# levendlee/np-modeling

Measured on AMD Instinct MI355X. Metric: fwd+bwd samples/sec, TransformerEncoder d=1024 seq=512, higher is better.
Workload: dtype f32; 1 GPU; TransformerEncoder fwd+bwd+SGD step, d_model=1024, heads=8, seq=512, hidden_units=4096, pre-norm, batch 256/GPU (BASELINE.json configs[4] per-GPU shard; global batch 256); global_batch=256, seq_len=512, parallelism=single GPU

## Files before the change

np_modeling_amd/csrc/npm_attn.hip:

```cpp
#include <algorithm>
#include <cmath>
#include <cstring>

#include "npm_mfma_tile.h"

namespace {

using npm_tile::f32x16;
using npm_tile::xcd_remap;

constexpr float LOG2E = 1.44269504088896340736f;
constexpr float LN2 = 0.69314718055994530942f;
constexpr int OOB = 0x7FFFFFFF;

struct MhaArgs {
    const float *q, *k, *v;
    long q_pitch, k_pitch, v_pitch;
    float *ctx;
    long ctx_pitch;
    float *lse;
    float *delta;
    long delta_sb, delta_sh;
    int delta_len;
    float *lse2;
    int sq_pad;
    const unsigned char *skip;
    long skip_sb, skip_sh;
    int skip_nkb;
    long skip_all;
    const float *dctx;
    long dctx_pitch;
    float *dq, *dk, *dv;
    long dq_pitch, dk_pitch, dv_pitch;
    const unsigned char *mask;
    long mask_sb, mask_sh, mask_sq;
    float *scores;
    int batch, heads, seq_q, seq_kv;
    int kv_heads;
    float scale;
    int q_tiles;
    int q_pair;
    int stagger;
    long long *trace;
};

template <int D>
struct Tile {
    static constexpr int CPR = D / 4;
    static constexpr int SWZ = (CPR < 16 ? CPR : 16) - 1;
    __host__ __device__ static constexpr int sw(int row) {
        return D >= 64 ? ((row & 15) ^ ((row & 4) << 1))
             : D == 32 ? (((row >> 1) & 1) | (((row >> 3) & 1) << 1) | (((row >> 2) & 1) << 2))
                       : (((row >> 3) & 1) << 1);
    }
    __host__ __device__ static constexpr int prow(int row) { return D <= 32 ? row ^ ((row >> 2) & 1) : row; }
    static constexpr int PIECE_ROWS = 256 / D;
    static constexpr int NG = D / 8;
    static constexpr int NB = NG < 8 ? NG : 8;
    static_assert(D == 16 || D == 32 || D == 64 || D == 128 || D == 256, "head dim (256: the dS tile of a 256-key block)");
    __device__ static __forceinline__ int chunk(int row, int c) { return prow(row) * D + ((c ^ sw(row)) << 2); }
    __device__ static __forceinline__ int elem(int row, int col) { return prow(row) * D + ((((col >> 2) ^ sw(row)) << 2) | (col & 3)); }
    __device__ static __forceinline__ unsigned src(int lane, int piece, long pitch) {
        const int row = prow(piece * PIECE_ROWS + lane / CPR);
        const int c = (lane % CPR) ^ sw(row);
        return (unsigned)((row * pitch + c * 4) * 4);
    }
    __device__ static __forceinline__ void row_bases(int l32, int half, int (&rb)[NB]) {
#pragma unroll
        for (int j = 0; j < NB; ++j) rb[j] = chunk(l32, 2 * j + half);
    }
    __device__ static constexpr int row_imm(int g) { return (g >> 3) * 64; }
    static constexpr int VEC = D >= 32 ? D / 32 : 1;
    __device__ static __forceinline__ void vec_bases(int half, int l32, int (&vb)[2][4]) {
        const int col = VEC * (D < 32 ? (l32 & (D - 1)) : l32);
#pragma unroll
        for (int par = 0; par < 2; ++par)
#pragma unroll
            for (int k = 0; k < 4; ++k) vb[par][k] = elem(4 * half + k + 8 * par, col);
    }
    __device__ static constexpr int vec_imm(int r) { return 16 * (r >> 3) * D; }
};

__device__ __forceinline__ float4 ld4(const float *p) { return *reinterpret_cast<const float4 *>(p); }
template <int VEC>
__device__ __forceinline__ void ldv(const float *p, float (&v)[4]) {
    if (VEC == 4) { const float4 x = ld4(p); v[0] = x.x; v[1] = x.y; v[2] = x.z; v[3] = x.w; }
    else if (VEC == 2) { const float2 x = *reinterpret_cast<const float2 *>(p); v[0] = x.x; v[1] = x.y; }
    else v[0] = p[0];
}
__device__ __forceinline__ float ld_stream(const float *p) { return __builtin_nontemporal_load(p); }
__device__ __forceinline__ float xhalf(float x) { return __shfl_xor(x, 32, 64); }
__device__ __forceinline__ float fast_exp2(float x) { return __builtin_amdgcn_exp2f(x); }

typedef unsigned u32x4_t __attribute__((ext_vector_type(4)));

__device__ __forceinline__ float4 buf_load4(__amdgpu_buffer_rsrc_t r, int voff) {
    const u32x4_t v = __builtin_amdgcn_raw_buffer_load_b128(r, voff, 0, 0);
    return make_float4(__uint_as_float(v.x), __uint_as_float(v.y), __uint_as_float(v.z), __uint_as_float(v.w));
}
__device__ __forceinline__ void buf_store4(__amdgpu_buffer_rsrc_t r, int voff, float a, float b, float c, float d) {
    u32x4_t v = {__float_as_uint(a), __float_as_uint(b), __float_as_uint(c), __float_as_uint(d)};
    __builtin_amdgcn_raw_buffer_store_b128(v, r, voff, 0, 0);
}
__device__ __forceinline__ __amdgpu_buffer_rsrc_t make_rsrc(const void *base, long bytes) {
    return __builtin_amdgcn_make_buffer_rsrc((void *)base, 0, (int)std::min<long>(std::max<long>(bytes, 0), 0x7FFFFFF0L), 0x00020000);
}

using npm_tile::i32x4_t;
using npm_tile::make_desc;
using npm_tile::lds_offset;
using npm_tile::dma_group;

#define MFMA(a, b, c) __builtin_amdgcn_mfma_f32_32x32x2f32((a), (b), (c), 0, 0, 0)

template <int STEPS, int READS, int MFMAS>
__device__ __forceinline__ void sched_pipeline() {
    __builtin_amdgcn_sched_group_barrier(0x100, READS, 0);
#pragma unroll
    for (int i = 0; i + 1 < STEPS; ++i) {
        __builtin_amdgcn_sched_group_barrier(0x100, READS, 0);
        __builtin_amdgcn_sched_group_barrier(0x008, MFMAS, 0);
    }
    __builtin_amdgcn_sched_group_barrier(0x008, MFMAS, 0);
}
#define PHASE_END() __builtin_amdgcn_sched_barrier(0)
#define FENCE() __builtin_amdgcn_sched_barrier(0)
#define STAMP(slot) do { if (tr) { FENCE(); tr[slot] = __builtin_amdgcn_s_memtime(); FENCE(); } } while (0)

__device__ __forceinline__ void zero16(f32x16 &x) {
#pragma unroll
    for (int e = 0; e < 16; ++e) x[e] = 0.f;
}

template <int D, bool MASK, bool SAVE, bool TRACE>
__global__ void __launch_bounds__(256, 2)
mha_fwd_kernel(const MhaArgs p) {
    using T = Tile<D>;
    constexpr int NG = D / 8, DT = (D + 31) / 32, VEC = T::VEC, TILE = 32 * D, PIECES = D / 8, PPW = (PIECES + 3) / 4;
    __shared__ __attribute__((aligned(16))) float smem[4 * TILE];

    const int tid = threadIdx.x, lane = tid & 63;
    const int wave = __builtin_amdgcn_readfirstlane(tid >> 6);
    long long *const blk_tr = (TRACE && p.trace && tid == 0) ? p.trace + (long)blockIdx.x * 16 : nullptr;
    if (blk_tr) blk_tr[9] = __builtin_amdgcn_s_memtime();
    const int l32 = lane & 31, half = lane >> 5;

    const int logical = xcd_remap(blockIdx.x, gridDim.x);
    const bool pairing = MASK && p.q_pair;
    const int units = pairing ? (p.q_tiles + 1) / 2 : p.q_tiles;
    const int unit = logical % units, bh = logical / units;
    const int b = bh / p.heads, h = bh - b * p.heads;
  for (int rep = 0; rep < (pairing ? 2 : 1); ++rep) {
    const int qt = rep == 0 ? unit : p.q_tiles - 1 - unit;
    if (rep == 1) {
        if (qt == unit) break;
// ... 672 lines not shown
                    S = MFMA(fa[g & 1].x, fk[g & 1].x, S);
                    S = MFMA(fa[g & 1].y, fk[g & 1].y, S);
                    S = MFMA(fa[g & 1].z, fk[g & 1].z, S);
                    S = MFMA(fa[g & 1].w, fk[g & 1].w, S);
                    FENCE();
                }
            }
            STAMP(1);
            constexpr int F0 = SAVED ? 0 : (NG & 1);
            zero16(dP);
#pragma unroll
            for (int g = 0; g < NG; ++g) {
                if (g + 1 < NG) fa[(F0 + g + 1) & 1] = ld4(tDO + rb[(g + 1) & 7] + T::row_imm(g + 1));
                else ldv<VEC>(tDO + vb[0][0], ea[0]);
                FENCE();
                dP = MFMA(fa[(F0 + g) & 1].x, vf[g].x, dP);
                dP = MFMA(fa[(F0 + g) & 1].y, vf[g].y, dP);
                dP = MFMA(fa[(F0 + g) & 1].z, vf[g].z, dP);
                dP = MFMA(fa[(F0 + g) & 1].w, vf[g].w, dP);
                FENCE();
            }
            unsigned char mk[16];
            if (MASK) {
                const int mvoff = kvok ? kvrow + 4 * half * (int)p.mask_sq : OOB;
#pragma unroll
                for (int r = 0; r < 16; ++r)
                    mk[r] = __builtin_amdgcn_raw_buffer_load_b8(rsrcM, mvoff, (q0 + (r & 3) + 8 * (r >> 2)) * (int)p.mask_sq, 0);
            }
            if (kb * 128 + 128 > p.seq_kv && !kvok) {
#pragma unroll
                for (int r = 0; r < 16; ++r) S[r] = -INFINITY;
            }
#pragma unroll
            for (int r = 0; r < 16; ++r) {
                const float pr = fast_exp2(fmaf((MASK && mk[r] == 0) ? -INFINITY : S[r], c, -Lr[r]));
                P[r] = pr;
                dS[r] = pr * (dP[r] - Dr[r]);
                sDS[ebs[(r >> 2) & 1][r & 3] + 8 * (r >> 2) * 128] = dS[r];
            }
            STAMP(2);
#pragma unroll
            for (int r = 0; r < 16; ++r) {
                if (r + 1 < 16) ldv<VEC>(tDO + vb[((r + 1) >> 2) & 1][(r + 1) & 3] + T::vec_imm(r + 1), ea[(r + 1) & 1]);
                FENCE();
#pragma unroll
                for (int t = 0; t < DT; ++t) dV[t] = MFMA(ea[r & 1][t], P[r], dV[t]);
                FENCE();
            }
            STAMP(3);
            asm volatile("s_waitcnt lgkmcnt(0)" ::: "memory");
            __builtin_amdgcn_s_barrier();
            asm volatile("" ::: "memory");
            STAMP(4);

            if (dq_wave) {
                float4 da[2];
                float dk4[2][4];
                da[0] = ld4(sDS + rbs[0]);
#pragma unroll
                for (int k = 0; k < 4; ++k) dk4[0][k] = sKB[ebk[0][k]];
#pragma unroll
                for (int g = 0; g < 16; ++g) {
                    if (g + 1 < 16) {
                        da[(g + 1) & 1] = ld4(sDS + rbs[(g + 1) & 7] + TS::row_imm(g + 1));
#pragma unroll
                        for (int k = 0; k < 4; ++k) dk4[(g + 1) & 1][k] = sKB[8 * (g + 1) * D + ebk[(g + 1) & 1][k]];
                    } else {
                        ldv<VEC>(tQ + vb[0][0], ea[0]);
                    }
                    if (g == 1) issue_half(nq, nxt, 0);
                    if (g == 9) issue_half(nq, nxt, 1);
                    FENCE();
                    acc = MFMA(dk4[g & 1][0], da[g & 1].x, acc);
                    acc = MFMA(dk4[g & 1][1], da[g & 1].y, acc);
                    acc = MFMA(dk4[g & 1][2], da[g & 1].z, acc);
                    acc = MFMA(dk4[g & 1][3], da[g & 1].w, acc);
                    FENCE();
                }
            } else {
                issue_half(nq, nxt, 0);
                issue_half(nq, nxt, 1);
                ldv<VEC>(tQ + vb[0][0], ea[0]);
            }
            STAMP(5);
            if (seam) {
                __builtin_amdgcn_s_barrier();
                asm volatile("" ::: "memory");
                issue_kblock(kb + 1);
                load_vfrag(kb + 1);
            }
#pragma unroll
            for (int r = 0; r < 16; ++r) {
                if (r + 1 < 16) ldv<VEC>(tQ + vb[((r + 1) >> 2) & 1][(r + 1) & 3] + T::vec_imm(r + 1), ea[(r + 1) & 1]);
                if ((r & 3) == 0 && 8 * (r >> 2) < D) {
                    const int g4 = r >> 2;
                    const u32x4_t v = {__float_as_uint(acc[r]), __float_as_uint(acc[r + 1]), __float_as_uint(acc[r + 2]), __float_as_uint(acc[r + 3])};
                    __builtin_amdgcn_raw_buffer_store_b128(v, rsrcDQw, dq_voff + 32 * g4, dq_tile, 0);
                }
                FENCE();
#pragma unroll
                for (int t = 0; t < DT; ++t) dK[t] = MFMA(ea[r & 1][t], dS[r], dK[t]);
                FENCE();
            }
            if (half == 0) { xs[l32] = lse_n * LOG2E; xs[32 + l32] = dlt_n; }
            in_flight = 4;
            ++it;
            STAMP(6);
            STAMP(7);
            FENCE();
        }
        if (blk_tr && kb == 0) blk_tr[11] = __builtin_amdgcn_s_memtime();
        if (SEAM_STORES == 0) asm volatile("s_waitcnt vmcnt(0)" ::: "memory");
#pragma unroll
        for (int r = 0; r < 16; ++r) {
            const int d0 = VEC * (4 * half + (r & 3) + 8 * (r >> 2));
            if (VEC * (8 * (r >> 2) + (r & 3)) < D) {
                const bool ok = kvok && d0 < D;
                const int offk = ok ? (int)((kvrow * p.dk_pitch + d0) * 4) : OOB, offv = ok ? (int)((kvrow * p.dv_pitch + d0) * 4) : OOB;
                if (VEC == 4) {
                    buf_store4(rsrcDK, offk, dK[0][r], dK[DT > 1 ? 1 : 0][r], dK[DT > 2 ? 2 : 0][r], dK[DT > 3 ? 3 : 0][r]);
                    buf_store4(rsrcDV, offv, dV[0][r], dV[DT > 1 ? 1 : 0][r], dV[DT > 2 ? 2 : 0][r], dV[DT > 3 ? 3 : 0][r]);
                } else {
#pragma unroll
                    for (int t = 0; t < DT; ++t) {
                        __builtin_amdgcn_raw_buffer_store_b32(__float_as_uint(dK[t][r]), rsrcDK, ok ? offk + 4 * t : OOB, 0, 0);
                        __builtin_amdgcn_raw_buffer_store_b32(__float_as_uint(dV[t][r]), rsrcDV, ok ? offv + 4 * t : OOB, 0, 0);
                    }
                }
            }
        }
    }
    if (blk_tr) {
        blk_tr[12] = __builtin_amdgcn_s_memtime();
        asm volatile("s_waitcnt vmcnt(0)" ::: "memory");
        blk_tr[13] = __builtin_amdgcn_s_memtime();
    }
}


template <bool TRACE>
__global__ void __launch_bounds__(512, 1)
mha_bwd16_kernel(const MhaArgs p) {
    constexpr int D = 128;
    using T = Tile<D>;
    constexpr int QTILE = 32 * D, KBLK = 128 * D, ROWS16 = 16 * D;
    __shared__ __attribute__((aligned(16))) float smem[KBLK + 4 * QTILE + 32 * 128];
    float *const sKB = smem, *const sQ = sKB + KBLK, *const sDO = sQ + 2 * QTILE, *const sDS = sDO + 2 * QTILE;

    const int tid = threadIdx.x, lane = tid & 63;
    const int wave = __builtin_amdgcn_readfirstlane(tid >> 6);
    const int l16 = lane & 15, kk = lane >> 4;
    const int bh = blockIdx.x;
    const int b = bh / p.heads, h = bh - b * p.heads;
    long long *const blk_tr = (TRACE && p.trace && tid == 0) ? p.trace + (long)blockIdx.x * 16 : nullptr;
    if (blk_tr) blk_tr[9] = __builtin_amdgcn_s_memtime();

    const auto descK = make_desc(p.k + (long)b * p.seq_kv * p.k_pitch + (h % p.kv_heads) * D, ((long)(p.seq_kv - 1) * p.k_pitch + D) * 4);
    const auto rsrcV = make_rsrc(p.v + (long)b * p.seq_kv * p.v_pitch + (h % p.kv_heads) * D, ((long)(p.seq_kv - 1) * p.v_pitch + D) * 4);
    const auto descQ = make_desc(p.q + (long)b * p.seq_q * p.q_pitch + h * D, ((long)(p.seq_q - 1) * p.q_pitch + D) * 4);
    const auto descDO = make_desc(p.dctx + (long)b * p.seq_q * p.dctx_pitch + h * D, ((long)(p.seq_q - 1) * p.dctx_pitch + D) * 4);
    const auto rsrcDQ = make_rsrc(p.dq + (long)b * p.seq_q * p.dq_pitch + h * D, ((long)(p.seq_q - 1) * p.dq_pitch + D) * 4);
    const auto rsrcDK = make_rsrc(p.dk + (long)b * p.seq_kv * p.dk_pitch + h * D, ((long)(p.seq_kv - 1) * p.dk_pitch + D) * 4);
    const auto rsrcDV = make_rsrc(p.dv + (long)b * p.seq_kv * p.dv_pitch + h * D, ((long)(p.seq_kv - 1) * p.dv_pitch + D) * 4);
    const auto rsrcNone = make_rsrc(p.dq, 0);
    const auto rsrcL = make_rsrc(p.lse2 + (long)bh * p.sq_pad, (long)p.sq_pad * 4);
    const auto rsrcDl = make_rsrc(p.delta + b * p.delta_sb + h * p.delta_sh, (long)p.delta_len * 4);
    const auto rsrcS = make_rsrc(p.scores + (long)bh * p.seq_q * p.seq_kv, (long)p.seq_q * p.seq_kv * 4);
    const int srow_bytes = p.seq_kv * 4;

    unsigned vq[2], vdo[2], vkb[8];
#pragma unroll
    for (int i = 0; i < 2; ++i) {
        vq[i] = T::src(lane, wave * 2 + i, p.q_pitch);
        vdo[i] = T::src(lane, wave * 2 + i, p.dctx_pitch);
    }
#pragma unroll
    for (int i = 0; i < 8; ++i) vkb[i] = T::src(lane, wave * 8 + i, p.k_pitch);
    const unsigned qstep = (unsigned)(32 * p.q_pitch * 4), dostep = (unsigned)(32 * p.dctx_pitch * 4);
    const unsigned lds_q = lds_offset(sQ + wave * 2 * 256), lds_do = lds_offset(sDO + wave * 2 * 256), lds_kb = lds_offset(sKB + wave * 8 * 256);

    int rb[4], vb[4], ws[4];
#pragma unroll
    for (int j = 0; j < 4; ++j) {
        rb[j] = T::chunk(l16, 4 * j + kk);
        vb[j] = T::elem(4 * kk + j, 4 * l16);
        ws[j] = T::elem(4 * kk + j, 16 * wave + l16);
    }

    const float c = p.scale * LOG2E;
    const int nqt = (p.seq_q + 31) / 32, nkb = (p.seq_kv + 127) / 128;
    const int kvl = 16 * wave + l16;
    const int dq_voff = (int)((l16 * p.dq_pitch + 16 * wave + 4 * kk) * 4);
    const int dq_sub = 16 * (int)p.dq_pitch * 4;

    float4 vf[8];
    int it = 0;
    dma_group<8>(descK, lds_kb, 0u, vkb);
    {
        const int row = kvl;
#pragma unroll
        for (int cc = 0; cc < 8; ++cc) {
            vf[cc] = buf_load4(rsrcV, row < p.seq_kv ? (int)((row * p.v_pitch + 16 * cc + 4 * kk) * 4) : OOB);
            vf[cc].x *= p.scale; vf[cc].y *= p.scale; vf[cc].z *= p.scale; vf[cc].w *= p.scale;
        }
    }
    dma_group<2>(descQ, lds_q, 0u, vq);
    dma_group<2>(descDO, lds_do, 0u, vdo);

    bool scale_pending = false;
    f32x4 Lr_n[2], Dr_n[2];
    auto load_rows = [&](int qfirst) {
#pragma unroll
        for (int t = 0; t < 2; ++t) {
            const u32x4_t l4 = __builtin_amdgcn_raw_buffer_load_b128(rsrcL, 16 * kk, (qfirst + 16 * t) * 4, 0);
            const u32x4_t d4 = __builtin_amdgcn_raw_buffer_load_b128(rsrcDl, 16 * kk, (qfirst + 16 * t) * 4, 0);
            Lr_n[t] = f32x4{__uint_as_float(l4.x), __uint_as_float(l4.y), __uint_as_float(l4.z), __uint_as_float(l4.w)};
            Dr_n[t] = f32x4{__uint_as_float(d4.x), __uint_as_float(d4.y), __uint_as_float(d4.z), __uint_as_float(d4.w)};
        }
    };
    load_rows(0);
    if (blk_tr) blk_tr[10] = __builtin_amdgcn_s_memtime();
    for (int kb = 0; kb < nkb; ++kb) {
        const int kvrow = kb * 128 + kvl;
        const bool kvok = kvrow < p.seq_kv;
        f32x4 dK[8], dV[8];
#pragma unroll
        for (int t = 0; t < 8; ++t) { dK[t] = f32x4{0.f, 0.f, 0.f, 0.f}; dV[t] = f32x4{0.f, 0.f, 0.f, 0.f}; }
        const auto rsrcOld = kb > 0 ? rsrcDQ : rsrcNone;
        const int svoff = kvok ? (kvrow + 4 * kk * p.seq_kv) * 4 : OOB;
        int in_flight = kb > 0 ? 18 : 0;

        for (int qt = 0; qt < nqt; ++qt) {
            long long *const tr = (TRACE && blk_tr && kb == (nkb > 1 ? 1 : 0) && qt == (nqt > 5 ? 5 : 0)) ? blk_tr : nullptr;
            STAMP(0);
            if (in_flight == 2) asm volatile("s_waitcnt vmcnt(2) ; npm:wait" ::: "memory");
            else if (in_flight == 18) asm volatile("s_waitcnt vmcnt(18) ; npm:wait" ::: "memory");
            else asm volatile("s_waitcnt vmcnt(0)" ::: "memory");
            asm volatile("s_waitcnt lgkmcnt(0)" ::: "memory");
            __builtin_amdgcn_s_barrier();
            asm volatile("" ::: "memory");
            if (scale_pending) {
#pragma unroll
                for (int cc = 0; cc < 8; ++cc) { vf[cc].x *= p.scale; vf[cc].y *= p.scale; vf[cc].z *= p.scale; vf[cc].w *= p.scale; }
                scale_pending = false;
            }
            STAMP(1);
            const bool seam = qt + 1 == nqt && kb + 1 < nkb;
            const int nq = qt + 1 < nqt ? qt + 1 : 0;
            const int cur = it & 1, nxt = cur ^ 1;
            const float *tQ = sQ + cur * QTILE, *tDO = sDO + cur * QTILE;
            const int q0 = 32 * qt;
            f32x4 Lr[2], Dr[2];
#pragma unroll
            for (int t = 0; t < 2; ++t) { Lr[t] = Lr_n[t]; Dr[t] = Dr_n[t]; }
            load_rows(32 * nq);
            f32x4 S[2], acc[2];
#pragma unroll
            for (int t = 0; t < 2; ++t)
#pragma unroll
                for (int r = 0; r < 4; ++r)
                    S[t][r] = __uint_as_float(__builtin_amdgcn_raw_buffer_load_b32(rsrcS, svoff, (q0 + 16 * t + r) * srow_bytes, 2));
            const int dq_tile = q0 * (int)p.dq_pitch * 4;
#pragma unroll
            for (int t = 0; t < 2; ++t) {
                const u32x4_t o = __builtin_amdgcn_raw_buffer_load_b128(rsrcOld, dq_voff, dq_tile + t * dq_sub, 0);
                acc[t] = f32x4{__uint_as_float(o.x), __uint_as_float(o.y), __uint_as_float(o.z), __uint_as_float(o.w)};
            }

            f32x4 dP[2] = {Dr[0], Dr[1]};
            float4 fa[2][2];
            fa[0][0] = ld4(tDO + rb[0]);
            fa[0][1] = ld4(tDO + rb[0] + ROWS16);
#pragma unroll
            for (int cc = 0; cc < 8; ++cc) {
                if (cc + 1 < 8) {
                    fa[(cc + 1) & 1][0] = ld4(tDO + rb[(cc + 1) & 3] + ((cc + 1) >> 2) * 64);
                    fa[(cc + 1) & 1][1] = ld4(tDO + rb[(cc + 1) & 3] + ((cc + 1) >> 2) * 64 + ROWS16);
                }
                FENCE();
#pragma unroll
                for (int t = 0; t < 2; ++t) {
                    dP[t] = MFMA16(fa[cc & 1][t].x, vf[cc].x, dP[t]);
                    dP[t] = MFMA16(fa[cc & 1][t].y, vf[cc].y, dP[t]);
                    dP[t] = MFMA16(fa[cc & 1][t].z, vf[cc].z, dP[t]);
                    dP[t] = MFMA16(fa[cc & 1][t].w, vf[cc].w, dP[t]);
                }
                FENCE();
            }
            STAMP(2);
            if (kb * 128 + 128 > p.seq_kv && !kvok) {
#pragma unroll
                for (int t = 0; t < 2; ++t)
#pragma unroll
                    for (int r = 0; r < 4; ++r) S[t][r] = -INFINITY;
            }
            f32x4 P[2], dS[2];
#pragma unroll
            for (int t = 0; t < 2; ++t)
#pragma unroll
                for (int r = 0; r < 4; ++r) {
                    const float pr = fast_exp2(fmaf(S[t][r], c, -Lr[t][r]));
                    P[t][r] = pr;
                    dS[t][r] = pr * dP[t][r];
                    sDS[ws[r] + t * ROWS16] = dS[t][r];
                }
            STAMP(3);
            float4 ea[2][2];
            ea[0][0] = ld4(tDO + vb[0]);
            ea[0][1] = ld4(tDO + vb[0] + 64);
#pragma unroll
            for (int st = 0; st < 8; ++st) {
                const int t = st >> 2, r = st & 3;
                if (st + 1 < 8) {
                    ea[(st + 1) & 1][0] = ld4(tDO + vb[(st + 1) & 3] + ((st + 1) >> 2) * ROWS16);
                    ea[(st + 1) & 1][1] = ld4(tDO + vb[(st + 1) & 3] + ((st + 1) >> 2) * ROWS16 + 64);
                }
                FENCE();
                const float4 e0 = ea[st & 1][0], e1 = ea[st & 1][1];
                dV[0] = MFMA16(e0.x, P[t][r], dV[0]); dV[1] = MFMA16(e0.y, P[t][r], dV[1]);
                dV[2] = MFMA16(e0.z, P[t][r], dV[2]); dV[3] = MFMA16(e0.w, P[t][r], dV[3]);
                dV[4] = MFMA16(e1.x, P[t][r], dV[4]); dV[5] = MFMA16(e1.y, P[t][r], dV[5]);
                dV[6] = MFMA16(e1.z, P[t][r], dV[6]); dV[7] = MFMA16(e1.w, P[t][r], dV[7]);
                FENCE();
            }
            STAMP(4);
            asm volatile("s_waitcnt lgkmcnt(0)" ::: "memory");
            __builtin_amdgcn_s_barrier();
            asm volatile("" ::: "memory");
            STAMP(5);

            float ak[2][4];
            float4 da[2][2];
#pragma unroll
            for (int s = 0; s < 4; ++s) ak[0][s] = sKB[ws[s]];
            da[0][0] = ld4(sDS + rb[0]);
            da[0][1] = ld4(sDS + rb[0] + ROWS16);
#pragma unroll
            for (int cc = 0; cc < 8; ++cc) {
                if (cc + 1 < 8) {
#pragma unroll
                    for (int s = 0; s < 4; ++s) ak[(cc + 1) & 1][s] = sKB[ws[s] + (cc + 1) * ROWS16];
                    da[(cc + 1) & 1][0] = ld4(sDS + rb[(cc + 1) & 3] + ((cc + 1) >> 2) * 64);
                    da[(cc + 1) & 1][1] = ld4(sDS + rb[(cc + 1) & 3] + ((cc + 1) >> 2) * 64 + ROWS16);
                }
                if (cc == 1) dma_group<2>(descQ, lds_q + nxt * QTILE * 4, nq * qstep, vq);
                if (cc == 5) dma_group<2>(descDO, lds_do + nxt * QTILE * 4, nq * dostep, vdo);
                FENCE();
#pragma unroll
                for (int t = 0; t < 2; ++t) {
                    acc[t] = MFMA16(ak[cc & 1][0], da[cc & 1][t].x, acc[t]);
                    acc[t] = MFMA16(ak[cc & 1][1], da[cc & 1][t].y, acc[t]);
                    acc[t] = MFMA16(ak[cc & 1][2], da[cc & 1][t].z, acc[t]);
                    acc[t] = MFMA16(ak[cc & 1][3], da[cc & 1][t].w, acc[t]);
                }
                FENCE();
            }
            STAMP(6);
            if (seam) {
                __builtin_amdgcn_s_barrier();
                asm volatile("" ::: "memory");
                dma_group<8>(descK, lds_kb, (unsigned)((kb + 1) * 128 * p.k_pitch * 4), vkb);
                const int row = (kb + 1) * 128 + kvl;
#pragma unroll
                for (int cc = 0; cc < 8; ++cc) vf[cc] = buf_load4(rsrcV, row < p.seq_kv ? (int)((row * p.v_pitch + 16 * cc + 4 * kk) * 4) : OOB);
                scale_pending = true;
            }
            ea[0][0] = ld4(tQ + vb[0]);
            ea[0][1] = ld4(tQ + vb[0] + 64);
#pragma unroll
            for (int st = 0; st < 8; ++st) {
                const int t = st >> 2, r = st & 3;
                if (st + 1 < 8) {
                    ea[(st + 1) & 1][0] = ld4(tQ + vb[(st + 1) & 3] + ((st + 1) >> 2) * ROWS16);
                    ea[(st + 1) & 1][1] = ld4(tQ + vb[(st + 1) & 3] + ((st + 1) >> 2) * ROWS16 + 64);
                }
                if (st == 0 || st == 4) {
                    const int tt = st >> 2;
                    const u32x4_t v = {__float_as_uint(acc[tt][0]), __float_as_uint(acc[tt][1]), __float_as_uint(acc[tt][2]), __float_as_uint(acc[tt][3])};
                    __builtin_amdgcn_raw_buffer_store_b128(v, rsrcDQ, dq_voff, dq_tile + tt * dq_sub, 0);
                }
                FENCE();
                const float4 e0 = ea[st & 1][0], e1 = ea[st & 1][1];
                dK[0] = MFMA16(e0.x, dS[t][r], dK[0]); dK[1] = MFMA16(e0.y, dS[t][r], dK[1]);
                dK[2] = MFMA16(e0.z, dS[t][r], dK[2]); dK[3] = MFMA16(e0.w, dS[t][r], dK[3]);
                dK[4] = MFMA16(e1.x, dS[t][r], dK[4]); dK[5] = MFMA16(e1.y, dS[t][r], dK[5]);
                dK[6] = MFMA16(e1.z, dS[t][r], dK[6]); dK[7] = MFMA16(e1.w, dS[t][r], dK[7]);
                FENCE();
            }
            in_flight = 2;
            ++it;
            FENCE();
            STAMP(7);
        }
#pragma unroll
        for (int x = 0; x < 2; ++x)
#pragma unroll
            for (int r = 0; r < 4; ++r) {
                const int d0 = 64 * x + 16 * kk + 4 * r;
                const int offk = kvok ? (int)((kvrow * p.dk_pitch + d0) * 4) : OOB, offv = kvok ? (int)((kvrow * p.dv_pitch + d0) * 4) : OOB;
                buf_store4(rsrcDK, offk, dK[4 * x][r], dK[4 * x + 1][r], dK[4 * x + 2][r], dK[4 * x + 3][r]);
                buf_store4(rsrcDV, offv, dV[4 * x][r], dV[4 * x + 1][r], dV[4 * x + 2][r], dV[4 * x + 3][r]);
            }
    }
    if (blk_tr) {
        blk_tr[12] = __builtin_amdgcn_s_memtime();
        asm volatile("s_waitcnt vmcnt(0)" ::: "memory");
        blk_tr[13] = __builtin_amdgcn_s_memtime();
    }
}

template <int D, bool MASK, bool SAVED>
__global__ void __launch_bounds__(512, D <= 32 ? 4 : 2)
mha_bwd8_kernel(const MhaArgs p) {
    using T = Tile<D>;
    constexpr int KG = D == 64 ? 2 : 1;
    constexpr int SP = 128 * KG;
    using TS = Tile<SP>;
    constexpr int NC = D / 16;
    constexpr int QTILE = 32 * D, KBLK = SP * D, ROWS16 = 16 * D, SROWS16 = 16 * SP, DSBUF = 32 * SP;
    constexpr int QP = D / 8, QPPW = QP >= 8 ? QP / 8 : 1, KPPW = D / 16 * KG;
    constexpr int VW = D >= 64 ? 4 : D / 16, NV = NC / VW;
    constexpr int DQT = NC == 8 ? 2 : 1;
    constexpr int NB = NC < 4 ? NC : 4;
    constexpr bool CTP = D < 64;
    constexpr bool SPREAD = NC == 1;
    constexpr int PQBUF = 8 * 32 * D;
    static_assert(!(MASK && SAVED), "saved scores carry the mask");
    __shared__ __attribute__((aligned(16))) float smem[KBLK + 4 * QTILE + (SPREAD ? DSBUF + 2 * PQBUF : 2 * DSBUF)];
    float *const sKB = smem, *const sQ = sKB + KBLK, *const sDO = sQ + 2 * QTILE, *const sDS = sDO + 2 * QTILE;
    float *const sPQ = sDS + DSBUF;

    const int tid = threadIdx.x, lane = tid & 63;
    const int wave = __builtin_amdgcn_readfirstlane(tid >> 6);
    const int l16 = lane & 15, kk = lane >> 4;
    const int bh = blockIdx.x;
    const int b = bh / p.heads, h = bh - b * p.heads;

    const auto descK = make_desc(p.k + (long)b * p.seq_kv * p.k_pitch + (h % p.kv_heads) * D, ((long)(p.seq_kv - 1) * p.k_pitch + D) * 4);
    const auto rsrcV = make_rsrc(p.v + (long)b * p.seq_kv * p.v_pitch + (h % p.kv_heads) * D, ((long)(p.seq_kv - 1) * p.v_pitch + D) * 4);
    const auto descQ = make_desc(p.q + (long)b * p.seq_q * p.q_pitch + h * D, ((long)(p.seq_q - 1) * p.q_pitch + D) * 4);
    const auto descDO = make_desc(p.dctx + (long)b * p.seq_q * p.dctx_pitch + h * D, ((long)(p.seq_q - 1) * p.dctx_pitch + D) * 4);
    const auto rsrcDQ = make_rsrc(p.dq + (long)b * p.seq_q * p.dq_pitch + h * D, ((long)(p.seq_q - 1) * p.dq_pitch + D) * 4);
    const auto rsrcDK = make_rsrc(p.dk + (long)b * p.seq_kv * p.dk_pitch + h * D, ((long)(p.seq_kv - 1) * p.dk_pitch + D) * 4);
    const auto rsrcDV = make_rsrc(p.dv + (long)b * p.seq_kv * p.dv_pitch + h * D, ((long)(p.seq_kv - 1) * p.dv_pitch + D) * 4);
    const auto rsrcNone = make_rsrc(p.dq, 0);
    const auto rsrcL = make_rsrc(p.lse2 + (long)bh * p.sq_pad, (long)p.sq_pad * 4);
    const auto rsrcDl = make_rsrc(p.delta + b * p.delta_sb + h * p.delta_sh, (long)p.delta_len * 4);
    const auto rsrcS = make_rsrc(SAVED ? p.scores + (long)bh * p.seq_q * p.seq_kv : nullptr, SAVED ? (long)p.seq_q * p.seq_kv * 4 : 0);
    const int srow_bytes = p.seq_kv * 4;
    const auto rsrcM = make_rsrc(MASK ? p.mask + b * p.mask_sb + h * p.mask_sh : nullptr, MASK ? (long)(p.seq_q - 1) * p.mask_sq + p.seq_kv : 0);

    unsigned vq[QPPW], vdo[QPPW], vkb[KPPW];
#pragma unroll
    for (int i = 0; i < QPPW; ++i) {
        vq[i] = T::src(lane, wave * QPPW + i, p.q_pitch);
        vdo[i] = T::src(lane, wave * QPPW + i, p.dctx_pitch);
    }
#pragma unroll
    for (int i = 0; i < KPPW; ++i) vkb[i] = T::src(lane, wave * KPPW + i, p.k_pitch);
    const bool q_owner = QP >= 8 || wave < QP;
    const unsigned qstep = (unsigned)(32 * p.q_pitch * 4), dostep = (unsigned)(32 * p.dctx_pitch * 4);
    const unsigned lds_q = lds_offset(sQ + wave * QPPW * 256), lds_do = lds_offset(sDO + wave * QPPW * 256), lds_kb = lds_offset(sKB + wave * KPPW * 256);
    auto issue_q = [&](int qt, int stage) { if (q_owner) dma_group<QPPW>(descQ, lds_q + stage * QTILE * 4, (unsigned)qt * qstep, vq); };
    auto issue_do = [&](int qt, int stage) { if (q_owner) dma_group<QPPW>(descDO, lds_do + stage * QTILE * 4, (unsigned)qt * dostep, vdo); };

    int rb[NB], vb[4], rbS[4], wsS[4], wsK[4];
    const int dqs = NC == 8 ? wave : wave % NC;
    const int dqh = NC == 8 ? 0 : wave / NC;
    const bool dq_wave = NC == 8 || wave < 2 * NC;
#pragma unroll
    for (int j = 0; j < NB; ++j) rb[j] = T::chunk(l16, 4 * j + kk);
#pragma unroll
    for (int j = 0; j < 4; ++j) {
        vb[j] = T::elem(4 * kk + j, VW * l16);
        rbS[j] = TS::chunk(l16, 4 * j + kk);
        wsS[j] = TS::elem(4 * kk + j, 16 * wave + l16);
        wsK[j] = T::elem(4 * kk + j, 16 * dqs + l16);
    }
    const float *const sKW = sKB + 16 * wave * D;

    const float c = p.scale * LOG2E;
    const int nqt = (p.seq_q + 31) / 32, nkb = (p.seq_kv + SP - 1) / SP;
    const int kvl = 16 * wave + l16;
    const int dq_voff = SPREAD ? (int)(((tid >> 4) * p.dq_pitch + (tid & 15)) * 4)
                               : (int)((l16 * p.dq_pitch + 16 * dqs + 4 * kk) * 4);
    const int dq_sub = 16 * (int)p.dq_pitch * 4;
    static_assert(!SPREAD || D == 16, "the partial tile's swizzle is written for 16-float rows");
    const int own_ds = TS::chunk(l16, 4 * wave + kk), own_pq = wave * 32 * D + l16 * D + ((kk ^ ((l16 >> 1) & 3)) << 2);
    int own_k[4];
#pragma unroll
    for (int s = 0; s < 4; ++s) own_k[s] = T::elem(4 * kk + s, l16) + 16 * wave * D;

    const unsigned char *const sk = p.skip ? p.skip + b * p.skip_sb + h * p.skip_sh : nullptr;
    auto load_tiles = [&](int kb, int &bytes) -> unsigned long {
        if (!sk) return ~0ul;
        int ln = lane;
        asm volatile("" : "+v"(ln));
        bytes = 0;
#pragma unroll
        for (int kg = 0; kg < KG; ++kg) {
            const int k128 = KG * kb + kg;
            if (ln < nqt && k128 < p.skip_nkb) {
                int bb = (int)sk[(long)ln * p.skip_nkb + k128];
                if (MASK && p.skip_all) bb |= (int)sk[p.skip_all + (long)ln * p.skip_nkb + k128] << 8;
                bytes |= bb << (16 * kg);
            }
        }
        const unsigned long any = __builtin_amdgcn_ballot_w64((bytes & 0x00ff00ff) != 0);
        return any ? any : 1ul;
    };
    auto first_tile = [&](unsigned long act) -> int { return sk ? __builtin_ctzl(act) : 0; };
    auto next_tile = [&](unsigned long act, int from) -> int {
        if (!sk) return from < nqt ? from : -1;
        if (from >= 64) return -1;
        const unsigned long m = act >> from;
        return m ? from + __builtin_ctzl(m) : -1;
    };

    float4 vf[KG][NC];
    auto load_vfrag = [&](int kb) {
#pragma unroll
        for (int kg = 0; kg < KG; ++kg) {
            const int row = kb * SP + 128 * kg + kvl;
#pragma unroll
            for (int cc = 0; cc < NC; ++cc) {
                vf[kg][cc] = buf_load4(rsrcV, row < p.seq_kv ? (int)((row * p.v_pitch + 16 * cc + 4 * kk) * 4) : OOB);
                vf[kg][cc].x *= p.scale; vf[kg][cc].y *= p.scale; vf[kg][cc].z *= p.scale; vf[kg][cc].w *= p.scale;
            }
        }
    };

    int cur_bytes = 0x00ff00ff, nxt_bytes = 0x00ff00ff;
    unsigned long act = load_tiles(0, cur_bytes);
    unsigned long written = 0;
    dma_group<KPPW>(descK, lds_kb, 0u, vkb);
    load_vfrag(0);
    {
        const int q_first = first_tile(act);
        issue_q(q_first, 0);
        issue_do(q_first, 0);
    }
    int j = 0;
    int n_inflight = 0;

    f32x4 dK[KG][NC], dV[KG][NC], P[2], dS[KG][2];
    auto dq_phase = [&](int tile, int buf, const f32x4 (&oldq)[DQT]) __attribute__((always_inline)) {
        if constexpr (SPREAD) {
            const float *pp = sPQ + buf * PQBUF + ((tid & ~15) | ((((tid >> 2) ^ (tid >> 5)) & 3) << 2) | (tid & 3));
            float part[8];
#pragma unroll
            for (int w = 0; w < 8; ++w) part[w] = pp[w * 32 * D];
            float sum = oldq[0][0];
#pragma unroll
            for (int w = 0; w < 8; ++w) sum += part[w];
            __builtin_amdgcn_raw_buffer_store_b32(__float_as_uint(sum), rsrcDQ, dq_voff, tile * 32 * (int)p.dq_pitch * 4, 0);
        } else if (dq_wave) {
            const float *tS = sDS + buf * DSBUF + (NC == 8 ? 0 : dqh * SROWS16);
            f32x4 acc[DQT];
#pragma unroll
            for (int t = 0; t < DQT; ++t) acc[t] = oldq[t];
            float ak[2][4];
// ... 790 lines not shown
```

Measured before the change: 3392 samples/s.

## Peel last q-tile in bwd16 attention kernel and hoist seam loads

Turns the q-tile loop body into a lambda that is instantiated separately for the final tile, so the seam logic becomes compile-time. The next block's V fragment loads move earlier, into the last tile after the dP phase, and dV is stored from inside the last tile instead of after the loop. The LDS reads of K fragments are issued before the barrier and repeated only when the K block has just been refreshed. The aim is to overlap seam-time global traffic with compute and shorten the critical path at block boundaries. It also adds trace stamps (enlarging the trace stride) and a fixed vmcnt(14) wait that may be tuned too tightly or loosely.

```diff
diff --git a/np_modeling_amd/csrc/npm_attn.hip b/np_modeling_amd/csrc/npm_attn.hip
--- a/np_modeling_amd/csrc/npm_attn.hip
+++ b/np_modeling_amd/csrc/npm_attn.hip
@@ -1,6 +1,7 @@
 #include <algorithm>
 #include <cmath>
 #include <cstring>
+#include <type_traits>
 
 #include "npm_mfma_tile.h"
 
@@ -979,7 +980,8 @@
     const int l16 = lane & 15, kk = lane >> 4;
     const int bh = blockIdx.x;
     const int b = bh / p.heads, h = bh - b * p.heads;
-    long long *const blk_tr = (TRACE && p.trace && tid == 0) ? p.trace + (long)blockIdx.x * 16 : nullptr;
+    long long *const blk_tr = (TRACE && p.trace && tid == 0) ? p.trace + (long)blockIdx.x * 32 : nullptr;
+#define SEAM_STAMP(cond, slot) do { if (TRACE && blk_tr && (cond)) { FENCE(); blk_tr[slot] = __builtin_amdgcn_s_memtime(); FENCE(); } } while (0)
     if (blk_tr) blk_tr[9] = __builtin_amdgcn_s_memtime();
 
     const auto descK = make_desc(p.k + (long)b * p.seq_kv * p.k_pitch + (h % p.kv_heads) * D, ((long)(p.seq_kv - 1) * p.k_pitch + D) * 4);
@@ -1055,11 +1057,15 @@
         for (int t = 0; t < 8; ++t) { dK[t] = f32x4{0.f, 0.f, 0.f, 0.f}; dV[t] = f32x4{0.f, 0.f, 0.f, 0.f}; }
         const auto rsrcOld = kb > 0 ? rsrcDQ : rsrcNone;
         const int svoff = kvok ? (kvrow + 4 * kk * p.seq_kv) * 4 : OOB;
+        const int dv_voff = kvok ? (int)((kvrow * p.dv_pitch + 16 * kk) * 4) : OOB;
         int in_flight = kb > 0 ? 18 : 0;
 
-        for (int qt = 0; qt < nqt; ++qt) {
+        auto tile = [&](const int qt, auto last_tag) __attribute__((always_inline)) {
+            constexpr bool LAST = decltype(last_tag)::value;
             long long *const tr = (TRACE && blk_tr && kb == (nkb > 1 ? 1 : 0) && qt == (nqt > 5 ? 5 : 0)) ? blk_tr : nullptr;
             STAMP(0);
+            SEAM_STAMP(LAST && kb == 0 && nkb > 1, 23);
+            SEAM_STAMP(kb == 1 && qt == 0, 19);
             if (in_flight == 2) asm volatile("s_waitcnt vmcnt(2) ; npm:wait" ::: "memory");
             else if (in_flight == 18) asm volatile("s_waitcnt vmcnt(18) ; npm:wait" ::: "memory");
             else asm volatile("s_waitcnt vmcnt(0)" ::: "memory");
@@ -1072,8 +1078,9 @@
                 scale_pending = false;
             }
             STAMP(1);
-            const bool seam = qt + 1 == nqt && kb + 1 < nkb;
-            const int nq = qt + 1 < nqt ? qt + 1 : 0;
+            SEAM_STAMP(kb == 1 && qt == 0, 20);
+            constexpr bool seam = LAST;
+            const int nq = LAST ? 0 : qt + 1;
             const int cur = it & 1, nxt = cur ^ 1;
             const float *tQ = sQ + cur * QTILE, *tDO = sDO + cur * QTILE;
             const int q0 = 32 * qt;
@@ -1082,12 +1089,12 @@
             for (int t = 0; t < 2; ++t) { Lr[t] = Lr_n[t]; Dr[t] = Dr_n[t]; }
             load_rows(32 * nq);
             f32x4 S[2], acc[2];
+            const int dq_tile = q0 * (int)p.dq_pitch * 4;
 #pragma unroll
             for (int t = 0; t < 2; ++t)
 #pragma unroll
                 for (int r = 0; r < 4; ++r)
                     S[t][r] = __uint_as_float(__builtin_amdgcn_raw_buffer_load_b32(rsrcS, svoff, (q0 + 16 * t + r) * srow_bytes, 2));
-            const int dq_tile = q0 * (int)p.dq_pitch * 4;
 #pragma unroll
             for (int t = 0; t < 2; ++t) {
                 const u32x4_t o = __builtin_amdgcn_raw_buffer_load_b128(rsrcOld, dq_voff, dq_tile + t * dq_sub, 0);
@@ -1115,6 +1122,13 @@
                 FENCE();
             }
             STAMP(2);
+            SEAM_STAMP(kb == 1 && qt == 0, 21);
+            if constexpr (seam) {
+                const int row = (kb + 1) * 128 + kvl;
+#pragma unroll
+                for (int cc = 0; cc < 8; ++cc) vf[cc] = buf_load4(rsrcV, row < p.seq_kv ? (int)((row * p.v_pitch + 16 * cc + 4 * kk) * 4) : OOB);
+                scale_pending = true;
+            }
             if (kb * 128 + 128 > p.seq_kv && !kvok) {
 #pragma unroll
                 for (int t = 0; t < 2; ++t)
@@ -1132,6 +1146,7 @@
                     sDS[ws[r] + t * ROWS16] = dS[t][r];
                 }
             STAMP(3);
+            SEAM_STAMP(kb == 1 && qt == 0, 22);
             float4 ea[2][2];
             ea[0][0] = ld4(tDO + vb[0]);
             ea[0][1] = ld4(tDO + vb[0] + 64);
@@ -1151,15 +1166,30 @@
                 FENCE();
             }
             STAMP(4);
+            if constexpr (LAST) {
+#pragma unroll
+                for (int x = 0; x < 2; ++x)
+#pragma unroll
+                    for (int r = 0; r < 4; ++r) {
+                        const u32x4_t v = {__float_as_uint(dV[4 * x][r]), __float_as_uint(dV[4 * x + 1][r]), __float_as_uint(dV[4 * x + 2][r]), __float_as_uint(dV[4 * x + 3][r])};
+                        __builtin_amdgcn_raw_buffer_store_b128(v, rsrcDV, dv_voff, (64 * x + 4 * r) * 4, 0);
+                    }
+            }
+            asm volatile("s_waitcnt vmcnt(14) ; npm:wait" ::: "memory");
+            float ak[2][4];
+            const bool k_fresh = kb > 0 && qt == 0;
+#pragma unroll
+            for (int s = 0; s < 4; ++s) ak[0][s] = sKB[ws[s]];
             asm volatile("s_waitcnt lgkmcnt(0)" ::: "memory");
             __builtin_amdgcn_s_barrier();
             asm volatile("" ::: "memory");
             STAMP(5);
 
-            float ak[2][4];
             float4 da[2][2];
-#pragma unroll
-            for (int s = 0; s < 4; ++s) ak[0][s] = sKB[ws[s]];
+            if (k_fresh) {
+#pragma unroll
+                for (int s = 0; s < 4; ++s) ak[0][s] = sKB[ws[s]];
+            }
             da[0][0] = ld4(sDS + rb[0]);
             da[0][1] = ld4(sDS + rb[0] + ROWS16);
 #pragma unroll
@@ -1183,14 +1213,13 @@
                 FENCE();
             }
             STAMP(6);
-            if (seam) {
+            SEAM_STAMP(kb == 0 && seam && nkb > 1, 16);
+            if (seam && kb + 1 < nkb) {
                 __builtin_amdgcn_s_barrier();
                 asm volatile("" ::: "memory");
+                SEAM_STAMP(kb == 0, 17);
                 dma_group<8>(descK, lds_kb, (unsigned)((kb + 1) * 128 * p.k_pitch * 4), vkb);
-                const int row = (kb + 1) * 128 + kvl;
-#pragma unroll
-                for (int cc = 0; cc < 8; ++cc) vf[cc] = buf_load4(rsrcV, row < p.seq_kv ? (int)((row * p.v_pitch + 16 * cc + 4 * kk) * 4) : OOB);
-                scale_pending = true;
+                SEAM_STAMP(kb == 0, 18);
             }
             ea[0][0] = ld4(tQ + vb[0]);
             ea[0][1] = ld4(tQ + vb[0] + 64);
@@ -1218,15 +1247,17 @@
             ++it;
             FENCE();
             STAMP(7);
-        }
+            SEAM_STAMP(kb == 1 && qt == 0, 24);
+        };
+        for (int qt = 0; qt + 1 < nqt; ++qt) tile(qt, std::false_type{});
+        tile(nqt - 1, std::true_type{});
 #pragma unroll
         for (int x = 0; x < 2; ++x)
 #pragma unroll
             for (int r = 0; r < 4; ++r) {
                 const int d0 = 64 * x + 16 * kk + 4 * r;
-                const int offk = kvok ? (int)((kvrow * p.dk_pitch + d0) * 4) : OOB, offv = kvok ? (int)((kvrow * p.dv_pitch + d0) * 4) : OOB;
+                const int offk = kvok ? (int)((kvrow * p.dk_pitch + d0) * 4) : OOB;
                 buf_store4(rsrcDK, offk, dK[4 * x][r], dK[4 * x + 1][r], dK[4 * x + 2][r], dK[4 * x + 3][r]);
-                buf_store4(rsrcDV, offv, dV[4 * x][r], dV[4 * x + 1][r], dV[4 * x + 2][r], dV[4 * x + 3][r]);
             }
     }
     if (blk_tr) {
@@ -1234,6 +1265,7 @@
         asm volatile("s_waitcnt vmcnt(0)" ::: "memory");
         blk_tr[13] = __builtin_amdgcn_s_memtime();
     }
+#undef SEAM_STAMP
 }
 
 template <int D, bool MASK, bool SAVED>
```

After: 3394 samples/s, median of 2. Within noise of the previous version (+0.1%).
